# RubensBenevides/Point-Cloud-Registration-with-Global-Refinement

Measured on AMD Instinct MI355X. Metric: point-cloud pairs registered/sec (200k pts, 3 GICP scales), higher is better.
Workload: dtype f32 points+search, f64 normal equations (SURVEY 8a fp column)

## Files before the change

point-cloud-registration-with-global-refinement_amd/csrc/pcr_api.hip:

```cpp
#include <cmath>
#include <cstring>
#include <cstdlib>
#include <cstdio>
#include <atomic>
#include <mutex>
#include <thread>
#include <vector>
#include "pcr_octree.h"

extern "C" int pcr_version(void) { return 220; }

PcrOptions &pcr_options() {
    static PcrOptions o;
    static std::once_flag once;
    std::call_once(once, []() {
        if (const char *e = getenv("PCR_KNN_WAVE")) o.knn_wave = atoi(e);
        if (const char *e = getenv("PCR_KNNW_BUDGET")) o.knnw_budget = atoi(e);
        if (const char *e = getenv("PCR_FENCE_PREP")) o.fence_prep = atoi(e);
        if (getenv("PCR_ICP_VERIFY")) o.icp_verify = 1;
        if (const char *e = getenv("PCR_SPFH_FLOAT64")) o.spfh_float64 = atoi(e);
        if (const char *e = getenv("PCR_RADIUS_LIST_SELECT")) o.radius_list_select = atoi(e);
        if (const char *e = getenv("PCR_FEATNN_MUTUAL")) o.featnn_mutual = atoi(e);
        if (const char *e = getenv("PCR_ICP_SCALES")) o.icp_scales = atoi(e);
        if (const char *e = getenv("PCR_SEARCH_SORT_QUERIES")) o.search_sort_queries = atoi(e);
        if (const char *e = getenv("PCR_FPS_FORM")) o.fps_form = atoi(e);
        if (const char *e = getenv("PCR_FPS_WGS")) o.fps_wgs = atoi(e);
        if (const char *e = getenv("PCR_FPS_TIMEOUT")) o.fps_timeout = atoi(e);
        if (const char *e = getenv("PCR_NFL_FORM")) o.nfl_form = atoi(e);
    });
    return o;
}
PcrCounters &pcr_counters() { static PcrCounters c; return c; }
extern "C" long long pcr_counter(const char *name, int reset) {
    if (!name) return -1;
    PcrCounters &c = pcr_counters();
    std::atomic<long long> *v = !strcmp(name, "fgr_group_barrier_timeouts") ? &c.fgr_group_barrier_timeouts : !strcmp(name, "fgr_group_pool_overflows") ? &c.fgr_group_pool_overflows
                               : !strcmp(name, "fgr_group_pairs_redone_alone") ? &c.fgr_group_pairs_redone_alone : nullptr;
    if (!v) return -1;
    return reset ? v->exchange(0) : v->load();
}
extern "C" int pcr_set_option(const char *name, long long value) {
    if (!name) return PCR_EINVAL;
    PcrOptions &o = pcr_options();
    if (!strcmp(name, "knn_wave")) { o.knn_wave = (int)value; return PCR_OK; }
    if (!strcmp(name, "knnw_budget")) { o.knnw_budget = (int)value; return PCR_OK; }
    if (!strcmp(name, "fence_prep")) { o.fence_prep = (int)value; return PCR_OK; }
    if (!strcmp(name, "icp_verify")) { o.icp_verify = (int)value; return PCR_OK; }
    if (!strcmp(name, "spfh_float64")) { o.spfh_float64 = (int)value; return PCR_OK; }
    if (!strcmp(name, "radius_list_select")) { o.radius_list_select = (int)value; return PCR_OK; }
    if (!strcmp(name, "arena_poison")) { o.arena_poison = (int)value; return PCR_OK; }
    if (!strcmp(name, "featnn_mutual")) { o.featnn_mutual = (int)value; return PCR_OK; }
    if (!strcmp(name, "icp_scales")) { o.icp_scales = (int)value; return PCR_OK; }
    if (!strcmp(name, "search_sort_queries")) { o.search_sort_queries = (int)value; return PCR_OK; }
    if (!strcmp(name, "fps_form")) { o.fps_form = (int)value; return PCR_OK; }
    if (!strcmp(name, "fps_wgs")) { o.fps_wgs = (int)value; return PCR_OK; }
    if (!strcmp(name, "fps_timeout")) { o.fps_timeout = (int)value; return PCR_OK; }
    if (!strcmp(name, "nfl_form")) { o.nfl_form = (int)value; return PCR_OK; }
    return PCR_EINVAL;
}

extern "C" int pcr_create(int device, pcr_context **out) {
    if (!out) return PCR_EINVAL;
    *out = nullptr;
    int count = 0;
    if (hipGetDeviceCount(&count) != hipSuccess || count <= 0) return PCR_EHIP;
    if (device < 0 || device >= count) return PCR_EINVAL;
    if (hipSetDevice(device) != hipSuccess) return PCR_EHIP;
    pcr_context *ctx = new pcr_context();
    ctx->device = device;
    for (int i = 0; i < 2; i++)
        if (hipEventCreateWithFlags(&ctx->side_ev[i], hipEventDisableTiming) != hipSuccess) { delete ctx; return PCR_EHIP; }
    for (int i = 0; i < 8; i++)
        if (hipEventCreateWithFlags(&ctx->lane_ev[i], hipEventDisableTiming) != hipSuccess) { delete ctx; return PCR_EHIP; }
    ctx->pinned_cap = 1 << 16;
    if (hipHostMalloc((void **)&ctx->pinned, ctx->pinned_cap, hipHostMallocDefault) != hipSuccess) { delete ctx; return PCR_EHIP; }
    for (int i = 0; i < 2; i++)
        if (hipEventCreateWithFlags(&ctx->ev[i], hipEventDisableTiming) != hipSuccess) { delete ctx; return PCR_EHIP; }
    for (int i = 0; i < 2; i++)
        if (hipEventCreateWithFlags(&ctx->fence_ev[i], hipEventDisableTiming) != hipSuccess) { delete ctx; return PCR_EHIP; }
    ctx->fence_default = true;
// ... 667 lines not shown
        xyz[2 * g] = p.src_xyz; xyz[2 * g + 1] = p.tgt_xyz; nrm[2 * g] = p.src_normals; nrm[2 * g + 1] = p.tgt_normals;
        n[2 * g] = p.n_src; n[2 * g + 1] = p.n_tgt;
    }
    for (int c = 0; c < C; c++) total += (size_t)n_scales * ((size_t)n[c] + 512) * 1100 + pcr_sort_temp_bytes((size_t)n[c] * n_scales) + (size_t)n[c] * n_scales * 40 + (8u << 20);
    PCR_TRY(pcr_arena_reserve(ctx, total + (16u << 20)));
    std::vector<double> b6((size_t)C * 6);
    PCR_TRY(pcr_dev_bounds_batch(ctx, C, xyz.data(), n.data(), b6.data()));
    std::vector<double> dists((size_t)G * n_scales);
    for (int g = 0; g < G; g++) {
        if (radius_rule == 1) {
            const double *bs = &b6[12 * g], *bt = &b6[12 * g + 6];
            const double r1 = std::pow((bs[3] - bs[0]) * (bs[4] - bs[1]) * (bs[5] - bs[2]), 1.0 / 3.0), r2 = std::pow((bt[3] - bt[0]) * (bt[4] - bt[1]) * (bt[5] - bt[2]), 1.0 / 3.0);
            for (int s = 0; s < n_scales; s++) dists[(size_t)g * n_scales + s] = (r1 + r2) / 2 * std::pow(2.0, -(double)s);
        } else for (int s = 0; s < n_scales; s++) dists[(size_t)g * n_scales + s] = given_dists[s];
        for (int s = 0; s < 8; s++) px[g]->max_distances[s] = s < n_scales ? dists[(size_t)g * n_scales + s] : 0.0;
        for (int s = 0; s < n_scales; s++) if (!(dists[(size_t)g * n_scales + s] > 0.0)) { ctx->err = "max_correspondence_distance <= 0"; return PCR_EINVAL; }
    }
    int *cnt = arena<int>(ctx, (size_t)C * n_scales * 2);
    if (!cnt) return PCR_ENOMEM;
    std::vector<DevCloud> clean;
    bool declined = false;
    PCR_TRY(prep_group_scales(ctx, C, xyz.data(), nrm.data(), n.data(), b6.data(), voxels, n_scales, sor_k, sor_std, normal_k, clean, cnt, &declined));
    if (declined) return 1;
    std::vector<double> T((size_t)G * 16), md((size_t)G);
    std::vector<pcr_result> res((size_t)G);
    std::vector<int32_t *> match((size_t)G);
    for (int g = 0; g < G; g++) {
        memcpy(&T[16 * g], px[g]->base.init_T, 16 * sizeof(double));
        match[g] = arena<int32_t>(ctx, n[2 * g]);
        if (!match[g]) return PCR_ENOMEM;
    }
    int rc_all = 1;
    if (n_scales > 1 && pcr_options().icp_scales.load(std::memory_order_relaxed)) {
        std::vector<const DevCloud *> ss((size_t)G * n_scales), tt((size_t)G * n_scales);
        std::vector<double> mds((size_t)G * n_scales); std::vector<pcr_result> rall((size_t)G * n_scales);
        for (int g = 0; g < G; g++)
            for (int s = 0; s < n_scales; s++) {
                ss[(size_t)g * n_scales + s] = &clean[(size_t)(2 * g) * n_scales + s]; tt[(size_t)g * n_scales + s] = &clean[(size_t)(2 * g + 1) * n_scales + s];
                mds[(size_t)g * n_scales + s] = dists[(size_t)g * n_scales + s];
            }
        rc_all = pcr_dev_gicp_group_scales(ctx, G, n_scales, ss.data(), tt.data(), mds.data(), T.data(), params, rall.data(), match.data());
        if (rc_all != PCR_OK && rc_all != 1) return rc_all;
        if (rc_all == PCR_OK)
            for (int g = 0; g < G; g++) for (int s = 0; s < n_scales; s++) px[g]->base.records[s].icp = rall[(size_t)g * n_scales + s];
    }
    for (int s = 0; s < n_scales && rc_all == 1; s++) {
        std::vector<const DevCloud *> ss((size_t)G), tt((size_t)G);
        for (int g = 0; g < G; g++) { ss[g] = &clean[(size_t)(2 * g) * n_scales + s]; tt[g] = &clean[(size_t)(2 * g + 1) * n_scales + s]; md[g] = dists[(size_t)g * n_scales + s]; }
        PCR_TRY(pcr_dev_gicp_group(ctx, G, ss.data(), tt.data(), md.data(), T.data(), params, res.data(), match.data()));
        for (int g = 0; g < G; g++) { px[g]->base.records[s].icp = res[g]; memcpy(&T[16 * g], res[g].transformation, 16 * sizeof(double)); }
    }
    {
        std::vector<const int32_t *> mm; std::vector<const int *> nn; std::vector<int> cc; std::vector<int32_t *> oo;
        for (int g = 0; g < G; g++)
            if (px[g]->base.correspondences) {
                const DevCloud &last = clean[(size_t)(2 * g) * n_scales + n_scales - 1];
                mm.push_back(match[g]); nn.push_back(last.n); cc.push_back(last.cap); oo.push_back((int32_t *)px[g]->base.correspondences);
            }
        if (!mm.empty()) PCR_TRY(pcr_dev_compact_matches_batch(ctx, (int)mm.size(), mm.data(), nn.data(), cc.data(), oo.data()));
    }
    std::vector<int> h((size_t)C * n_scales * 2);
    PCR_HIP_CHECK(ctx, hipMemcpyAsync(h.data(), cnt, sizeof(int) * h.size(), hipMemcpyDeviceToHost, ctx->stream));
    PCR_HIP_CHECK(ctx, hipStreamSynchronize(ctx->stream));
    for (int g = 0; g < G; g++)
        for (int s = 0; s < n_scales; s++) {
            pcr_scale_record &r = px[g]->base.records[s];
            for (int w = 0; w < 2; w++) { r.n_voxel[w] = h[2 * ((size_t)(2 * g + w) * n_scales + s)]; r.n_clean[w] = h[2 * ((size_t)(2 * g + w) * n_scales + s) + 1]; }
        }
    return PCR_OK;
}

extern "C" int pcr_debug_scale_clouds(pcr_context *ctx, int count, const float *const *xyz, const float *const *normals, const int64_t *n, const double *voxels,
                                      int n_scales, int sor_k, double sor_std, int normal_k, int form, float *const *out_xyz, float *const *out_normals,
                                      int32_t *out_n_voxel, int32_t *out_n_clean) {
    return pcr_api_call(ctx, [&]() -> int {
    if (count < 1 || count > 64 || n_scales < 1 || n_scales > 8 || form < 0 || form > 2 || !xyz || !n || !voxels || !out_xyz || !out_normals || !out_n_voxel || !out_n_clean) return PCR_EINVAL;
    if (sor_k < 1 || !(sor_std > 0.0) || normal_k < 1) { ctx->err = "nb_neighbors < 1, std_ratio <= 0 or knn < 1"; return PCR_EINVAL; }
    for (int s = 0; s < n_scales; s++) if (!(voxels[s] > 0.0)) { ctx->err = "voxel_size <= 0"; return PCR_EINVAL; }
    const size_t K = (size_t)count * n_scales;
    size_t bytes = 16u << 20;
    for (int c = 0; c < count; c++) {
        if (n[c] <= 0 || n[c] > 0x7fffffff / 4 / n_scales || !xyz[c]) return PCR_EINVAL;
        for (int s = 0; s < n_scales; s++) if (!out_xyz[c * n_scales + s] || !out_normals[c * n_scales + s]) return PCR_EINVAL;
        bytes += (size_t)n_scales * ((size_t)n[c] + 512) * 1100 + pcr_sort_temp_bytes((size_t)n[c] * n_scales) + (size_t)n[c] * n_scales * 40 + (8u << 20);
        if (form == 0) bytes += (size_t)n_scales * 2 * pcr_scratch_bytes_for(n[c]);
    }
// ... 498 lines not shown
```

point-cloud-registration-with-global-refinement_amd/csrc/pcr_gicp.hip:

```cpp
#pragma clang fp contract(on)
#include <climits>
#include <cmath>
#include <cstring>
#include <cstdio>
#include <cstdlib>
#include <string>
#include <vector>
#include "pcr_octree.h"
#include "pcr_umeyama.h"
#include "pcr_solve6.h"

#include "pcr_icp_loop.h"
__global__ void k_icp_init(IcpState *st, IcpInit in) { d_icp_init(st, in); }
__global__ void k_icp_init_g(IcpState *st, const IcpInit *in) { d_icp_init(st + blockIdx.x, in[blockIdx.x]); }

template <int OPB>
__device__ static inline int oct_nn_query(const OctView &t, const OctMeta &m, OctStack<OPB> &stk, bool live, float qx, float qy, float qz,
                                          float r2cap, int hint, int ol, int oct, int ob, int *start_pt, float *d1_out, float *d2_out) {
    int best = -1; float bestd = r2cap, secd = r2cap;
    const bool active = live && m.nl >= 1;
    auto visit = [&](int first, int count) {
        int base = first; const int end = first + count;
        float d = 3.4e38f, dd = 3.4e38f; int id = -1;
        while (__ballot(base < end) != 0ull) {
// ... 835 lines not shown
    if (mode == ICP_MODE_P2PL && (p->loss < PCR_LOSS_L2 || p->loss > PCR_LOSS_GM)) { ctx->err = "unknown robust kernel (pcr_loss_kind)"; return PCR_EINVAL; }
    pcr_gicp_params g;
    memset(&g, 0, sizeof g);
    g.loss = mode == ICP_MODE_P2PL ? p->loss : PCR_LOSS_L2; g.loss_k = mode == ICP_MODE_P2PL ? p->loss_k : 1.0; g.epsilon = 1e-3;
    g.relative_fitness = p->relative_fitness; g.relative_rmse = p->relative_rmse; g.max_iteration = p->max_iteration;
    return icp_loop(ctx, src, tgt, max_dist, T0, &g, mode, out, match_dev);
}

int pcr_dev_colored_icp(pcr_context *ctx, const DevCloud *src, const DevCloud *tgt, double max_dist, const double *T0, const pcr_colored_icp_params *p,
                        const double *src_int, const double *tgt_int, const float4 *tgt_grad, pcr_result *out, int32_t *match_dev) {
    if (p->loss < PCR_LOSS_L2 || p->loss > PCR_LOSS_GM) { ctx->err = "unknown robust kernel (pcr_loss_kind)"; return PCR_EINVAL; }
    const double lambda = (p->lambda_geometric >= 0.0 && p->lambda_geometric <= 1.0) ? p->lambda_geometric : 0.968;
    pcr_gicp_params g;
    memset(&g, 0, sizeof g);
    g.loss = p->loss; g.loss_k = p->loss_k; g.epsilon = 1e-3;
    g.relative_fitness = p->relative_fitness; g.relative_rmse = p->relative_rmse; g.max_iteration = p->max_iteration;
    IcpColorArgs c;
    memset(&c, 0, sizeof c);
    c.tgt_grad = tgt_grad; c.tgt_int = tgt_int; c.src_int = src_int; c.sqrt_lg = std::sqrt(lambda); c.sqrt_lp = std::sqrt(1.0 - lambda);
    return icp_loop(ctx, src, tgt, max_dist, T0, &g, ICP_MODE_COLORED, out, match_dev, &c);
}

int pcr_dev_gicp_group(pcr_context *ctx, int G, const DevCloud *const *src, const DevCloud *const *tgt, const double *max_dists, const double *T0,
                       const pcr_gicp_params *p, pcr_result *out, int32_t *const *match_dev) {
    for (int g = 0; g < G; g++) if (!(max_dists[g] > 0.0)) { ctx->err = "max_correspondence_distance <= 0"; return PCR_EINVAL; }
    if (G < 1 || G > ICP_GROUP_MAX) { ctx->err = "GICP group size must be in 1..32"; return PCR_EINVAL; }
    for (int g = 0; g < G; g++) if (!src[g]->nrm || !tgt[g]->nrm) { ctx->err = "GICP needs normals on both clouds"; return PCR_EINVAL; }
    ArenaMark mark(ctx);
    const IcpSwitches &sw = icp_switches();
    int max_cap = 1;
    for (int g = 0; g < G; g++) max_cap = src[g]->cap > max_cap ? src[g]->cap : max_cap;
    const int tile_pts = fused_tile_points(ctx, max_cap, G);
    IcpGroupBuf buf;
    PCR_TRY(icp_group_buf(ctx, &buf));
    IcpArgs *args = buf.args;
    int nblin = 1, nbnn = 1, nbf = 1;
    IcpState *st = arena<IcpState>(ctx, G);
    if (!st) return PCR_ENOMEM;
    for (int g = 0; g < G; g++) {
        const int cap = src[g]->cap > 0 ? src[g]->cap : 1;
        const int tile_g = icp_group_tile(cap, tile_pts) ? icp_group_tile(cap, tile_pts) : tile_pts;
        const IcpGrids n = icp_grids(cap, tile_g);
        nblin = n.nblin > nblin ? n.nblin : nblin; nbnn = n.nbnn > nbnn ? n.nbnn : nbnn; nbf = n.nbf > nbf ? n.nbf : nbf;
        double *partials = arena<double>(ctx, (size_t)(n.nblin > n.nbf ? n.nblin : n.nbf) * NVP);
        int32_t *match = (match_dev && match_dev[g]) ? match_dev[g] : arena<int32_t>(ctx, cap);
        if (!partials || !match) return PCR_ENOMEM;
        IcpArgs &a = args[g]; memset(&a, 0, sizeof a);
        const double max_dist = max_dists[g];
        fill_args(a, src[g], tgt[g], max_dist, p, match, st + g, partials, 0);
        a.tile_rt = icp_group_tile(cap, tile_pts);
        a.ref = arena<float4>(ctx, cap); a.rbest = arena<int32_t>(ctx, cap); a.clist = arena<int4>(ctx, cap);
        if (!a.ref || !a.rbest || !a.clist) return PCR_ENOMEM;
        const double gg = icp_base_gap(max_dist);
        icp_set_search_cap(a, max_dist, gg);
        a.rs_minus_r = (float)gg;
        memcpy(buf.inits[g].T, T0 + 16 * g, sizeof buf.inits[g].T);
    }
    bool grid = false;
    if (sw.grid) {
        std::vector<int> levels((size_t)G); std::vector<GridView> views((size_t)G);
        for (int g = 0; g < G; g++) levels[g] = pcr_grid_level_for(tgt[g], std::sqrt((double)args[g].r2s));
        bool all = true;
        for (int g = 0; g < G; g++) all = all && levels[g] >= 0 && tgt[g]->cap > 0;
        if (all) {
            PCR_TRY(pcr_dev_build_grid_batch(ctx, tgt, levels.data(), G, views.data()));
            grid = true;
            for (int g = 0; g < G; g++) { args[g].grid = views[g]; grid = grid && views[g].tab != nullptr; }
            if (grid)
                for (int g = 0; g < G; g++)
                    icp_set_search_cap(args[g], max_dists[g], icp_gap_for_level(tgt[g], levels[g], max_dists[g], (double)args[g].rs_minus_r));
        }
    }
    if (nbf > 4096) { ctx->err = "GICP group: cloud too large for the fused iteration kernel"; return PCR_EINVAL; }
    PCR_HIP_CHECK(ctx, hipMemcpyAsync(buf.dargs, buf.args, buf.bytes, hipMemcpyHostToDevice, ctx->stream));
    const IcpArgs *dargs = buf.dargs;
    PCR_LAUNCH(ctx, k_icp_init_g, dim3(G), dim3(64), 0, ctx->stream, st, (const IcpInit *)buf.dinits);
    const int max_it = p ? p->max_iteration : 30;
    const bool byval = sw.byval && G <= ICP_BYVAL;
    IcpArgsB hb; memset(&hb, 0, sizeof hb);
    for (int g = 0; g < G && g < ICP_BYVAL; g++) hb.a[g] = args[g];
    auto one_kernel = [&](int launch_index) { return launch_index > 0 && sw.fused; };
    auto enqueue = [&](int launch_index) {
        if (one_kernel(launch_index)) {
            if (byval) PCR_FUSED_LAUNCH(ctx, k_icp_fused_b, grid, tile_pts, dim3(nbf, G), hb);
            else PCR_FUSED_LAUNCH(ctx, k_icp_fused_g, grid, tile_pts, dim3(nbf, G), dargs);
            return;
        }
        if (grid) PCR_LAUNCH(ctx, k_icp_nn_g<true>, dim3(nbnn, G), dim3(ICP_BS), 0, ctx->stream, dargs);
        else PCR_LAUNCH(ctx, k_icp_nn_g<false>, dim3(nbnn, G), dim3(ICP_BS), 0, ctx->stream, dargs);
        PCR_LAUNCH(ctx, k_icp_lin_g, dim3(nblin, G), dim3(LIN_BS), 0, ctx->stream, dargs);
    };
    const void *dargs_v = dargs;
    std::string now;
    { const int w[3] = {nbnn, nblin, nbf}; now.assign((const char *)w, sizeof w); if (byval) now.append((const char *)&hb, sizeof hb); }
    auto graph_for = [&](int which, int len, hipGraphExec_t *exec) -> int {
        const long long kv[6] = {0x47525550ll , G + (grid ? 1000 : 0) + (sw.fused ? 0 : 2000) + (byval ? 4000 : 0), tile_pts, len, which, (long long)(uintptr_t)dargs_v};
        const std::string key((const char *)kv, sizeof kv);
        auto launch_of = [&](int k) { return which == 0 ? k : len + k; };
        IcpGraph *hit = icp_graph_find(ctx, key);
        if (!hit) {
            size_t kernels = 0;
            for (int k = 0; k < len; k++) kernels += one_kernel(launch_of(k)) ? 1 : 2;
            PCR_TRY(icp_graph_capture(ctx, key, len, kernels, [&](int k) { enqueue(launch_of(k)); }, &hit));
            hit->baked = now;
        } else if (hit->baked != now) {
            size_t i = 0;
            for (int k = 0; k < len; k++) {
                const bool one = one_kernel(launch_of(k));
                for (int part = 0; part < (one ? 1 : 2); part++, i++) {
                    if (i >= hit->nodes.size()) { ctx->err = "GICP group: captured chunk shorter than its launch list"; return PCR_EHIP; }
                    hipKernelNodeParams np;
                    PCR_HIP_CHECK(ctx, hipGraphKernelNodeGetParams(hit->nodes[i], &np));
                    void *kp[1];
                    if (one) { np.gridDim = dim3(nbf, G); kp[0] = byval ? (void *)&hb : (void *)&dargs_v; }
                    else { np.gridDim = part == 0 ? dim3(nbnn, G) : dim3(nblin, G); kp[0] = (void *)&dargs_v; }
                    np.kernelParams = kp; np.extra = nullptr;
                    PCR_HIP_CHECK(ctx, hipGraphExecKernelNodeSetParams(hit->exec, hit->nodes[i], &np));
                }
            }
            hit->baked = now;
        }
        *exec = hit->exec;
        return PCR_OK;
    };
    auto issue = [&](int k, int c, bool ragged) -> int {
        hipGraphExec_t ge = nullptr;
        if (sw.graph && !ragged) PCR_TRY(graph_for(k == 0 ? 0 : 1, c, &ge));
        if (ge) PCR_HIP_CHECK(ctx, hipGraphLaunch(ge, ctx->stream));
        else for (int i = 0; i < c; i++) enqueue(k + i);
        return PCR_OK;
    };
    std::vector<IcpState> fin((size_t)G);
    auto judge = [&](const IcpState *s, int, int *next) -> int {
        bool all = true;
        for (int g = 0; g < G; g++) all = all && s[g].done;
        if (all) { fin.assign(s, s + G); *next = 0; return PCR_OK; }
        *next = 1;
        for (int g = 0; g < G; g++)
            if (!s[g].done) { const int l = icp_next_chunk(s[g], args[g].rel_fit, args[g].rel_rmse, sw.chunk, true); *next = l > *next ? l : *next; }
        return PCR_OK;
    };
    IcpPump pump;
    PCR_TRY(pump.init(ctx, st, G));
    PCR_TRY(pump.run(sw.chunk, max_it + 1, issue, judge));
    if (!pump.done) { ctx->err = "GICP group loop ended without a final state"; return PCR_EHIP; }
    PCR_HIP_CHECK(ctx, hipStreamSynchronize(ctx->stream));
    if (ctx->profiling) {
        int longest = 0;
        for (int g = 0; g < G; g++) { icp_prof_add_state(ctx, fin[g]); longest = fin[g].launches > longest ? fin[g].launches : longest; }
        PCR_TRY(pump.add_profile(longest));
    }
    for (int g = 0; g < G; g++) {
        state_to_result(fin[g], &out[g]);
        for (int k = 0; k < 16; k++) if (!std::isfinite(fin[g].T[k])) { ctx->err = "non-finite pose"; return PCR_ENUMERIC; }
    }
    return PCR_OK;
}

int pcr_dev_gicp_group_scales(pcr_context *ctx, int G, int S, const DevCloud *const *src, const DevCloud *const *tgt, const double *max_dists, const double *T0,
                              const pcr_gicp_params *p, pcr_result *out, int32_t *const *match_dev) {
    if (G < 1 || G > ICP_GROUP_MAX || S < 1 || S > 8) return 1;
    const IcpSwitches &sw = icp_switches();
    if (!sw.fused || !sw.grid) return 1;
    if (pcr_options().icp_verify.load(std::memory_order_relaxed)) return 1;
    for (int k = 0; k < G * S; k++) {
        if (!(max_dists[k] > 0.0)) { ctx->err = "max_correspondence_distance <= 0"; return PCR_EINVAL; }
        if (!src[k]->nrm || !tgt[k]->nrm) { ctx->err = "GICP needs normals on both clouds"; return PCR_EINVAL; }
        if (tgt[k]->cap <= 0) return 1;
    }
    int max_cap = 1;
    for (int k = 0; k < G * S; k++) max_cap = src[k]->cap > max_cap ? src[k]->cap : max_cap;
    const int tile_pts = fused_tile_points(ctx, max_cap, G);
    for (int k = 0; k < G * S; k++) {
        const int cap = src[k]->cap > 0 ? src[k]->cap : 1;
        const int tile_k = icp_group_tile(cap, tile_pts) ? icp_group_tile(cap, tile_pts) : tile_pts;
        if (tile_k != LIN_BS) return 1;
    }
    ArenaMark mark(ctx);
    std::vector<int> levels((size_t)G * S); std::vector<GridView> views((size_t)G * S);
    for (int k = 0; k < G * S; k++) {
        IcpArgs base;
        icp_set_search_cap(base, max_dists[k], icp_base_gap(max_dists[k]));
        levels[k] = pcr_grid_level_for(tgt[k], std::sqrt((double)base.r2s));
        if (levels[k] < 0) return 1;
    }
    PCR_TRY(pcr_dev_build_grid_batch(ctx, tgt, levels.data(), G * S, views.data()));
    for (int k = 0; k < G * S; k++) if (!views[k].tab) return 1;
    IcpGroupBuf buf;
    PCR_TRY(icp_group_buf(ctx, &buf));
    IcpArgs *dargs = buf.dargs;
    const void *dargs_v = dargs;
    IcpState *st = arena<IcpState>(ctx, G), *hist = arena<IcpState>(ctx, (size_t)G * S);
    IcpArgs *all_dev = arena<IcpArgs>(ctx, (size_t)G * S);
    if (!st || !hist || !all_dev) return PCR_ENOMEM;
    std::vector<IcpArgs> all((size_t)G * S);
    int nbf = 1;
    for (int g = 0; g < G; g++) {
        int cap_g = 1, rows_g = 1;
        for (int s_ = 0; s_ < S; s_++) {
            const int cap = src[g * S + s_]->cap > 0 ? src[g * S + s_]->cap : 1;
            const int f_ = icp_grids(cap, LIN_BS).nbf;
            nbf = f_ > nbf ? f_ : nbf; cap_g = cap > cap_g ? cap : cap_g; rows_g = f_ > rows_g ? f_ : rows_g;
        }
        double *partials = arena<double>(ctx, (size_t)rows_g * NVP);
        int32_t *match = (match_dev && match_dev[g]) ? match_dev[g] : arena<int32_t>(ctx, cap_g);
        float4 *ref = arena<float4>(ctx, cap_g); int32_t *rbest = arena<int32_t>(ctx, cap_g); int4 *clist = arena<int4>(ctx, cap_g);
        if (!partials || !match || !ref || !rbest || !clist) return PCR_ENOMEM;
        for (int s_ = 0; s_ < S; s_++) {
            const int k = g * S + s_;
            IcpArgs &a = all[k]; memset(&a, 0, sizeof a);
            fill_args(a, src[k], tgt[k], max_dists[k], p, match, st + g, partials, 0);
            a.tile_rt = icp_group_tile(src[k]->cap > 0 ? src[k]->cap : 1, tile_pts);
            a.ref = ref; a.rbest = rbest; a.clist = clist;
            icp_set_search_cap(a, max_dists[k], icp_gap_for_level(tgt[k], levels[k], max_dists[k], icp_base_gap(max_dists[k])));
            a.grid = views[k];
            a.ms_args = all_dev + (size_t)g * S; a.ms_self = dargs + g; a.ms_hist = hist + (size_t)g * S; a.ms_scales = S; a.ms_index = s_;
        }
    }
    if (nbf > 4096) return 1;
    std::vector<IcpArgs> first((size_t)G); std::vector<IcpInit> inits((size_t)G);
    for (int g = 0; g < G; g++) { first[g] = all[(size_t)g * S]; memcpy(inits[g].T, T0 + 16 * g, sizeof inits[g].T); }
    PCR_HIP_CHECK(ctx, hipMemcpyAsync(all_dev, all.data(), sizeof(IcpArgs) * all.size(), hipMemcpyHostToDevice, ctx->stream));
    PCR_HIP_CHECK(ctx, hipMemcpyAsync(dargs, first.data(), sizeof(IcpArgs) * (size_t)G, hipMemcpyHostToDevice, ctx->stream));
    PCR_HIP_CHECK(ctx, hipMemcpyAsync(buf.dinits, inits.data(), sizeof(IcpInit) * (size_t)G, hipMemcpyHostToDevice, ctx->stream));
    PCR_LAUNCH(ctx, k_icp_init_g, dim3(G), dim3(64), 0, ctx->stream, st, (const IcpInit *)buf.dinits);
    auto enqueue_fused = [&](int) { PCR_LAUNCH(ctx, (k_icp_fused_g<LIN_BS, true>), dim3(nbf, G), dim3(FUSED_BS), 0, ctx->stream, (const IcpArgs *)dargs); };
    auto issue = [&](int, int c, bool) -> int {
        IcpGraph *hit = nullptr;
        if (sw.graph) {
            const long long kv[6] = {0x47525053ll , G, LIN_BS, c, nbf, (long long)(uintptr_t)dargs_v};
            const std::string key((const char *)kv, sizeof kv);
            hit = icp_graph_find(ctx, key);
            if (!hit) PCR_TRY(icp_graph_capture(ctx, key, c, 0, enqueue_fused, &hit));
        }
        if (hit) PCR_HIP_CHECK(ctx, hipGraphLaunch(hit->exec, ctx->stream));
        else for (int i = 0; i < c; i++) enqueue_fused(i);
        return PCR_OK;
    };
    const int max_it = p ? p->max_iteration : 30;
    const long long launch_limit = (long long)S * ((long long)max_it + 2) + 4 * sw.chunk + 64;
    IcpPump pump;
    int live_launches = 0;
    auto judge = [&](const IcpState *s, int upto, int *next) -> int {
        bool all_done = true;
        *next = 1;
        for (int g = 0; g < G; g++) {
            if (s[g].done) continue;
            all_done = false;
            const int l = icp_next_chunk(s[g], all[(size_t)g * S].rel_fit, all[(size_t)g * S].rel_rmse, sw.chunk, true);
            *next = l > *next ? l : *next;
        }
        if (all_done) { *next = 0; return PCR_OK; }
        live_launches = upto;
        if (pump.launched > launch_limit) { ctx->err = "GICP group loop (all scales) did not end"; return PCR_EHIP; }
        return PCR_OK;
    };
    PCR_TRY(pump.init(ctx, st, G));
    PCR_TRY(pump.run(sw.chunk, INT_MAX, issue, judge));
    if (!pump.done) { ctx->err = "GICP group loop ended without a final state"; return PCR_EHIP; }
// ... 155 lines not shown
```

point-cloud-registration-with-global-refinement_amd/csrc/pcr_icp_loop.h:

```cpp
#pragma once
#include <cmath>
#include <cstring>
#include <string>
#include <vector>
#include "pcr_octree.h"
#include "pcr_umeyama.h"
#include "pcr_solve6.h"

#define ICP_BS 256
#define NV 30
#define NVP 32
#define LIN_BS 512
#define LIN_MAX_BLOCKS 128

enum { ICP_MODE_GICP = 0, ICP_MODE_EVAL = 1, ICP_MODE_GICP_COV = 2, ICP_MODE_P2PL = 3, ICP_MODE_P2P = 4, ICP_MODE_P2P_SCALED = 5, ICP_MODE_COLORED = 6, ICP_MODE_VGICP = 7,
       ICP_MODE_NDT = 8 };

struct IcpState {
    double T[16];
    double fitness, rmse;
    double sums[NVP];
    long long count;
    int iter;
    int launches;
// ... 255 lines not shown
    if (ctx->icp_graphs.size() >= 48) {
        PCR_HIP_CHECK(ctx, hipStreamSynchronize(ctx->stream));
        (void)hipGraphExecDestroy(ctx->icp_graphs[0].exec);
        if (ctx->icp_graphs[0].graph) (void)hipGraphDestroy(ctx->icp_graphs[0].graph);
        ctx->icp_graphs.erase(ctx->icp_graphs.begin());
    }
    owner.g = nullptr;
    ctx->icp_graphs.push_back(std::move(e));
    *out = &ctx->icp_graphs.back();
    return PCR_OK;
}

struct IcpPump {
    pcr_context *ctx = nullptr;
    const IcpState *st_dev = nullptr; size_t slot_bytes = 0;
    IcpState *slots[2] = {nullptr, nullptr};
    int cur = 0, prev = -1;
    int launched = 0;
    bool done = false;
    std::vector<int> chunk_first, chunk_last;

    int init(pcr_context *c, const IcpState *states_dev, int G) {
        ctx = c; st_dev = states_dev; slot_bytes = sizeof(IcpState) * (size_t)G;
        if (2 * slot_bytes > ctx->pinned_cap) { ctx->err = "ICP loop: pinned window too small"; return PCR_ENOMEM; }
        slots[0] = (IcpState *)ctx->pinned; slots[1] = (IcpState *)(ctx->pinned + slot_bytes);
        return PCR_OK;
    }
    template <class Issue, class Judge>
    int run(int first_len, int total, Issue &&issue, Judge &&judge) {
        int want = first_len;
        for (;;) {
            const int room = total - launched, c = room < want ? (room > 0 ? room : 0) : want;
            if (c > 0) {
                const size_t n = chunk_first.size();
                if (ctx->profiling) {
                    while (ctx->prof_events.size() < 2 * (n + 1)) { hipEvent_t e; PCR_HIP_CHECK(ctx, hipEventCreate(&e)); ctx->prof_events.push_back(e); }
                    PCR_HIP_CHECK(ctx, hipEventRecord(ctx->prof_events[2 * n], ctx->stream));
                }
                PCR_TRY(issue(launched, c, c != want));
                if (ctx->profiling) PCR_HIP_CHECK(ctx, hipEventRecord(ctx->prof_events[2 * n + 1], ctx->stream));
                chunk_first.push_back(launched); chunk_last.push_back(launched + c);
                launched += c;
                PCR_HIP_CHECK(ctx, hipMemcpyAsync(slots[cur], st_dev, slot_bytes, hipMemcpyDeviceToHost, ctx->stream));
                PCR_HIP_CHECK(ctx, hipEventRecord(ctx->ev[cur], ctx->stream));
            }
            if (prev >= 0) {
                PCR_HIP_CHECK(ctx, hipEventSynchronize(ctx->ev[prev]));
// ... 19 lines not shown
```

point-cloud-registration-with-global-refinement_amd/csrc/pcr_internal.h:

```cpp
#pragma once
#include <hip/hip_runtime.h>
#include <stdint.h>
#include <string>
#include <mutex>
#include <cstring>
#include <vector>
#include <atomic>
#include "../../include/pcr_hip.h"

struct PcrOptions { std::atomic<int> knn_wave{-1}, knnw_budget{80}, fence_prep{0}, icp_verify{0}, spfh_float64{0}, radius_list_select{1}, arena_poison{0}, featnn_mutual{1}, icp_scales{1}, search_sort_queries{-1}, fps_form{-1}, fps_wgs{0}, fps_timeout{-1}, nfl_form{1}; };
PcrOptions &pcr_options();
struct PcrCounters { std::atomic<long long> fgr_group_barrier_timeouts{0}, fgr_group_pool_overflows{0}, fgr_group_pairs_redone_alone{0}; };
PcrCounters &pcr_counters();
#define PCR_GROUP_FORMS_MAX_POINTS 400000


struct IcpGraph {
    std::string key;
    hipGraphExec_t exec = nullptr;
    hipGraph_t graph = nullptr;
    std::vector<hipGraphNode_t> nodes;
    std::string baked;
};

struct pcr_context {
    int device = 0;
    hipStream_t stream = nullptr;
    hipStream_t own_stream = nullptr;
    hipStream_t side_stream = nullptr;
    hipStream_t side_stream2 = nullptr;
    hipEvent_t side_ev[2] = {nullptr, nullptr};
    hipEvent_t lane_ev[8] = {};
    char *arena = nullptr;
    size_t arena_cap = 0, arena_off = 0;
    char *aux = nullptr;
// ... 184 lines not shown
                                   double max_dist, const double *T, pcr_result *result, int32_t *correspondences);

size_t pcr_feature_nn_scratch_bytes(int64_t n0, int64_t n1, int prune_mode = -1);
int pcr_feature_nn_mutual(pcr_context *ctx, const float *f0, int n0, const float *f1, int n1, int32_t *out_1to0, int32_t *out_0to1,
                          int prune_mode ,
                          int mutual_only = 0 );

int pcr_feature_nn_mutual_batch(pcr_context *ctx, int G, const float *const *f0, const int *n0, const float *const *f1, const int *n1, int32_t *const *out_1to0,
                                int32_t *const *out_0to1, const int **overflow_dev, int mutual_only = 0);

size_t pcr_feature_corres_scratch_bytes(int64_t ns, int64_t nt);
int pcr_feature_corres(pcr_context *ctx, const float *src_feat, int ns, const float *tgt_feat, int nt, int mutual_filter, int min_rows, int32_t *corres, int64_t *n_out);

int pcr_corres_check(pcr_context *ctx, const int32_t *corres, int64_t n_corres, int64_t n_src, int64_t n_tgt);

struct IcpOutputs { pcr_result res; };
int pcr_dev_gicp(pcr_context *ctx, const DevCloud *src, const DevCloud *tgt, double max_dist, const double *T0,
                 const pcr_gicp_params *p, pcr_result *out, int32_t *match_dev );
int pcr_dev_icp(pcr_context *ctx, const DevCloud *src, const DevCloud *tgt, double max_dist, const double *T0,
                const pcr_icp_params *p, pcr_result *out, int32_t *match_dev );
int pcr_dev_colored_icp(pcr_context *ctx, const DevCloud *src, const DevCloud *tgt, double max_dist, const double *T0, const pcr_colored_icp_params *p,
                        const double *src_int, const double *tgt_int, const float4 *tgt_grad, pcr_result *out, int32_t *match_dev );
void pcr_icp_loop_switches(int *chunk, bool *graph);
int pcr_dev_gicp_group_scales(pcr_context *ctx, int G, int S, const DevCloud *const *src , const DevCloud *const *tgt, const double *max_dists , const double *T0 ,
                              const pcr_gicp_params *p, pcr_result *out , int32_t *const *match_dev );
int pcr_dev_gicp_group(pcr_context *ctx, int G, const DevCloud *const *src, const DevCloud *const *tgt, const double *max_dists , const double *T0 ,
                       const pcr_gicp_params *p, pcr_result *out , int32_t *const *match_dev );
int pcr_dev_linearize_once(pcr_context *ctx, const DevCloud *src, const DevCloud *tgt, double max_dist, const double *T,
                           const pcr_gicp_params *p, double *JTJ36, double *JTr6, double *stats3, int32_t *match_dev);
int pcr_dev_evaluate(pcr_context *ctx, const DevCloud *src, const DevCloud *tgt, double max_dist, const double *T,
                     pcr_result *out, int32_t *match_dev, double *info36 );
int pcr_dev_evaluate_group(pcr_context *ctx, int G, const DevCloud *const *src, const DevCloud *const *tgt, double max_dist, const double *T ,
                           pcr_result *out , int32_t *const *match_dev );
int pcr_dev_compact_matches(pcr_context *ctx, const int32_t *match, const int *n, int cap, const uint32_t *src_perm,
                            const uint32_t *tgt_perm, int32_t *corr_out, int64_t *n_corr);
```

Measured before the change: 725.3.

## Size GICP group grids from live point counts and drop converged pairs

The post-prep point counts are now copied asynchronously into a pinned window right after prep. The GICP group paths poll that window and, once the counts have landed, shrink the fused-kernel grid width from the allocated capacity to the actual point count. In the per-scale path with by-value args, pairs that have converged are also removed from the launch rows. Graph nodes get their grid dimensions updated, alternating between two cached graphs, and new counters track launches, dispatched workgroups and live tiles. The aim is fewer idle workgroups over capacity padding and finished pairs, at the cost of extra graph updates, host polling of volatile memory, and dependence on the pinned-window layout.

```diff
diff --git a/point-cloud-registration-with-global-refinement_amd/csrc/pcr_api.hip b/point-cloud-registration-with-global-refinement_amd/csrc/pcr_api.hip
--- a/point-cloud-registration-with-global-refinement_amd/csrc/pcr_api.hip
+++ b/point-cloud-registration-with-global-refinement_amd/csrc/pcr_api.hip
@@ -27,6 +27,7 @@
         if (const char *e = getenv("PCR_FPS_WGS")) o.fps_wgs = atoi(e);
         if (const char *e = getenv("PCR_FPS_TIMEOUT")) o.fps_timeout = atoi(e);
         if (const char *e = getenv("PCR_NFL_FORM")) o.nfl_form = atoi(e);
+        if (const char *e = getenv("PCR_ICP_LIVE_GRID")) o.icp_live_grid = atoi(e);
     });
     return o;
 }
@@ -35,7 +36,8 @@
     if (!name) return -1;
     PcrCounters &c = pcr_counters();
     std::atomic<long long> *v = !strcmp(name, "fgr_group_barrier_timeouts") ? &c.fgr_group_barrier_timeouts : !strcmp(name, "fgr_group_pool_overflows") ? &c.fgr_group_pool_overflows
-                               : !strcmp(name, "fgr_group_pairs_redone_alone") ? &c.fgr_group_pairs_redone_alone : nullptr;
+                               : !strcmp(name, "fgr_group_pairs_redone_alone") ? &c.fgr_group_pairs_redone_alone : !strcmp(name, "icp_group_launches") ? &c.icp_group_launches
+                               : !strcmp(name, "icp_group_workgroups_dispatched") ? &c.icp_group_workgroups_dispatched : !strcmp(name, "icp_group_tiles_live") ? &c.icp_group_tiles_live : nullptr;
     if (!v) return -1;
     return reset ? v->exchange(0) : v->load();
 }
@@ -56,6 +58,7 @@
     if (!strcmp(name, "fps_wgs")) { o.fps_wgs = (int)value; return PCR_OK; }
     if (!strcmp(name, "fps_timeout")) { o.fps_timeout = (int)value; return PCR_OK; }
     if (!strcmp(name, "nfl_form")) { o.nfl_form = (int)value; return PCR_OK; }
+    if (!strcmp(name, "icp_live_grid")) { o.icp_live_grid = (int)value; return PCR_OK; }
     return PCR_EINVAL;
 }
 
@@ -769,6 +772,11 @@
     bool declined = false;
     PCR_TRY(prep_group_scales(ctx, C, xyz.data(), nrm.data(), n.data(), b6.data(), voxels, n_scales, sor_k, sor_std, normal_k, clean, cnt, &declined));
     if (declined) return 1;
+    const size_t n_cnt = (size_t)C * n_scales * 2;
+    if (n_cnt * sizeof(int) > PCR_PINNED_COUNTS_BYTES || ctx->pinned_cap < 2 * PCR_PINNED_COUNTS_BYTES) { ctx->err = "GICP group: pinned window too small for the counts"; return PCR_ENOMEM; }
+    volatile int *h = (volatile int *)(ctx->pinned + ctx->pinned_cap - PCR_PINNED_COUNTS_BYTES);
+    for (size_t k = 0; k < n_cnt; k++) h[k] = -1;
+    PCR_HIP_CHECK(ctx, hipMemcpyAsync((void *)h, cnt, sizeof(int) * n_cnt, hipMemcpyDeviceToHost, ctx->stream));
     std::vector<double> T((size_t)G * 16), md((size_t)G);
     std::vector<pcr_result> res((size_t)G);
     std::vector<int32_t *> match((size_t)G);
@@ -786,7 +794,8 @@
                 ss[(size_t)g * n_scales + s] = &clean[(size_t)(2 * g) * n_scales + s]; tt[(size_t)g * n_scales + s] = &clean[(size_t)(2 * g + 1) * n_scales + s];
                 mds[(size_t)g * n_scales + s] = dists[(size_t)g * n_scales + s];
             }
-        rc_all = pcr_dev_gicp_group_scales(ctx, G, n_scales, ss.data(), tt.data(), mds.data(), T.data(), params, rall.data(), match.data());
+        const IcpHostCounts hc{h + 1, 4 * n_scales, 2};
+        rc_all = pcr_dev_gicp_group_scales(ctx, G, n_scales, ss.data(), tt.data(), mds.data(), T.data(), params, rall.data(), match.data(), &hc);
         if (rc_all != PCR_OK && rc_all != 1) return rc_all;
         if (rc_all == PCR_OK)
             for (int g = 0; g < G; g++) for (int s = 0; s < n_scales; s++) px[g]->base.records[s].icp = rall[(size_t)g * n_scales + s];
@@ -794,7 +803,8 @@
     for (int s = 0; s < n_scales && rc_all == 1; s++) {
         std::vector<const DevCloud *> ss((size_t)G), tt((size_t)G);
         for (int g = 0; g < G; g++) { ss[g] = &clean[(size_t)(2 * g) * n_scales + s]; tt[g] = &clean[(size_t)(2 * g + 1) * n_scales + s]; md[g] = dists[(size_t)g * n_scales + s]; }
-        PCR_TRY(pcr_dev_gicp_group(ctx, G, ss.data(), tt.data(), md.data(), T.data(), params, res.data(), match.data()));
+        const IcpHostCounts hc{h + 2 * s + 1, 4 * n_scales, 0};
+        PCR_TRY(pcr_dev_gicp_group(ctx, G, ss.data(), tt.data(), md.data(), T.data(), params, res.data(), match.data(), &hc));
         for (int g = 0; g < G; g++) { px[g]->base.records[s].icp = res[g]; memcpy(&T[16 * g], res[g].transformation, 16 * sizeof(double)); }
     }
     {
@@ -804,11 +814,11 @@
                 const DevCloud &last = clean[(size_t)(2 * g) * n_scales + n_scales - 1];
                 mm.push_back(match[g]); nn.push_back(last.n); cc.push_back(last.cap); oo.push_back((int32_t *)px[g]->base.correspondences);
             }
-        if (!mm.empty()) PCR_TRY(pcr_dev_compact_matches_batch(ctx, (int)mm.size(), mm.data(), nn.data(), cc.data(), oo.data()));
-    }
-    std::vector<int> h((size_t)C * n_scales * 2);
-    PCR_HIP_CHECK(ctx, hipMemcpyAsync(h.data(), cnt, sizeof(int) * h.size(), hipMemcpyDeviceToHost, ctx->stream));
-    PCR_HIP_CHECK(ctx, hipStreamSynchronize(ctx->stream));
+        if (!mm.empty()) {
+            PCR_TRY(pcr_dev_compact_matches_batch(ctx, (int)mm.size(), mm.data(), nn.data(), cc.data(), oo.data()));
+            PCR_HIP_CHECK(ctx, hipStreamSynchronize(ctx->stream));
+        }
+    }
     for (int g = 0; g < G; g++)
         for (int s = 0; s < n_scales; s++) {
             pcr_scale_record &r = px[g]->base.records[s];
diff --git a/point-cloud-registration-with-global-refinement_amd/csrc/pcr_gicp.hip b/point-cloud-registration-with-global-refinement_amd/csrc/pcr_gicp.hip
--- a/point-cloud-registration-with-global-refinement_amd/csrc/pcr_gicp.hip
+++ b/point-cloud-registration-with-global-refinement_amd/csrc/pcr_gicp.hip
@@ -881,12 +881,14 @@
 }
 
 int pcr_dev_gicp_group(pcr_context *ctx, int G, const DevCloud *const *src, const DevCloud *const *tgt, const double *max_dists, const double *T0,
-                       const pcr_gicp_params *p, pcr_result *out, int32_t *const *match_dev) {
+                       const pcr_gicp_params *p, pcr_result *out, int32_t *const *match_dev, const IcpHostCounts *counts) {
     for (int g = 0; g < G; g++) if (!(max_dists[g] > 0.0)) { ctx->err = "max_correspondence_distance <= 0"; return PCR_EINVAL; }
     if (G < 1 || G > ICP_GROUP_MAX) { ctx->err = "GICP group size must be in 1..32"; return PCR_EINVAL; }
     for (int g = 0; g < G; g++) if (!src[g]->nrm || !tgt[g]->nrm) { ctx->err = "GICP needs normals on both clouds"; return PCR_EINVAL; }
     ArenaMark mark(ctx);
     const IcpSwitches &sw = icp_switches();
+    const bool live_grid = counts && counts->n && pcr_options().icp_live_grid.load(std::memory_order_relaxed) != 0;
+    std::vector<int> cap_of((size_t)G), tile_of((size_t)G), tiles_of((size_t)G), wide_of((size_t)G);
     int max_cap = 1;
     for (int g = 0; g < G; g++) max_cap = src[g]->cap > max_cap ? src[g]->cap : max_cap;
     const int tile_pts = fused_tile_points(ctx, max_cap, G);
@@ -900,6 +902,7 @@
         const int cap = src[g]->cap > 0 ? src[g]->cap : 1;
         const int tile_g = icp_group_tile(cap, tile_pts) ? icp_group_tile(cap, tile_pts) : tile_pts;
         const IcpGrids n = icp_grids(cap, tile_g);
+        cap_of[g] = cap; tile_of[g] = tile_g; tiles_of[g] = (cap + tile_g - 1) / tile_g; wide_of[g] = n.nbf;
         nblin = n.nblin > nblin ? n.nblin : nblin; nbnn = n.nbnn > nbnn ? n.nbnn : nbnn; nbf = n.nbf > nbf ? n.nbf : nbf;
         double *partials = arena<double>(ctx, (size_t)(n.nblin > n.nbf ? n.nblin : n.nbf) * NVP);
         int32_t *match = (match_dev && match_dev[g]) ? match_dev[g] : arena<int32_t>(ctx, cap);
@@ -936,12 +939,44 @@
     PCR_LAUNCH(ctx, k_icp_init_g, dim3(G), dim3(64), 0, ctx->stream, st, (const IcpInit *)buf.dinits);
     const int max_it = p ? p->max_iteration : 30;
     const bool byval = sw.byval && G <= ICP_BYVAL;
-    IcpArgsB hb; memset(&hb, 0, sizeof hb);
-    for (int g = 0; g < G && g < ICP_BYVAL; g++) hb.a[g] = args[g];
+    const bool live_rows = live_grid && byval;
+    std::vector<int> rows((size_t)G);
+    for (int g = 0; g < G; g++) rows[g] = g;
+    IcpArgsB hb;
+    int ny = G;
+    long long tiles_rows = 0;
+    auto set_rows = [&]() {
+        memset(&hb, 0, sizeof hb);
+        ny = (int)rows.size(); tiles_rows = 0; nbf = 8;
+        for (int j = 0; j < ny; j++) {
+            if (byval) hb.a[j] = args[rows[j]];
+            nbf = wide_of[rows[j]] > nbf ? wide_of[rows[j]] : nbf;
+            tiles_rows += tiles_of[rows[j]];
+        }
+    };
+    bool sized = false;
+    auto size_by_counts = [&]() {
+        if (!counts || !counts->n || sized) return;
+        for (int g = 0; g < G; g++) if (counts->n[(size_t)g * counts->pair_stride] < 0) return;
+        if (live_grid) { nblin = 1; nbnn = 1; }
+        for (int g = 0; g < G; g++) {
+            const int c = counts->n[(size_t)g * counts->pair_stride];
+            const int ns_g = c < 1 ? 1 : (c > cap_of[g] ? cap_of[g] : c);
+            const IcpGrids w = icp_grids(ns_g, tile_of[g]);
+            tiles_of[g] = (ns_g + tile_of[g] - 1) / tile_of[g];
+            if (!live_grid) continue;
+            wide_of[g] = w.nbf;
+            nblin = w.nblin > nblin ? w.nblin : nblin; nbnn = w.nbnn > nbnn ? w.nbnn : nbnn;
+        }
+        sized = true;
+        set_rows();
+    };
+    set_rows();
+    size_by_counts();
     auto one_kernel = [&](int launch_index) { return launch_index > 0 && sw.fused; };
     auto enqueue = [&](int launch_index) {
         if (one_kernel(launch_index)) {
-            if (byval) PCR_FUSED_LAUNCH(ctx, k_icp_fused_b, grid, tile_pts, dim3(nbf, G), hb);
+            if (byval) PCR_FUSED_LAUNCH(ctx, k_icp_fused_b, grid, tile_pts, dim3(nbf, ny), hb);
             else PCR_FUSED_LAUNCH(ctx, k_icp_fused_g, grid, tile_pts, dim3(nbf, G), dargs);
             return;
         }
@@ -950,10 +985,11 @@
         PCR_LAUNCH(ctx, k_icp_lin_g, dim3(nblin, G), dim3(LIN_BS), 0, ctx->stream, dargs);
     };
     const void *dargs_v = dargs;
-    std::string now;
-    { const int w[3] = {nbnn, nblin, nbf}; now.assign((const char *)w, sizeof w); if (byval) now.append((const char *)&hb, sizeof hb); }
+    int side = 0;
     auto graph_for = [&](int which, int len, hipGraphExec_t *exec) -> int {
-        const long long kv[6] = {0x47525550ll , G + (grid ? 1000 : 0) + (sw.fused ? 0 : 2000) + (byval ? 4000 : 0), tile_pts, len, which, (long long)(uintptr_t)dargs_v};
+        std::string now;
+        { const int w[4] = {nbnn, nblin, nbf, ny}; now.assign((const char *)w, sizeof w); if (byval) now.append((const char *)&hb, sizeof hb); }
+        const long long kv[6] = {0x47525550ll , G + (grid ? 1000 : 0) + (sw.fused ? 0 : 2000) + (byval ? 4000 : 0) + (live_grid ? 8000 + 8000 * side : 0), tile_pts, len, which, (long long)(uintptr_t)dargs_v};
         const std::string key((const char *)kv, sizeof kv);
         auto launch_of = [&](int k) { return which == 0 ? k : len + k; };
         IcpGraph *hit = icp_graph_find(ctx, key);
@@ -971,7 +1007,7 @@
                     hipKernelNodeParams np;
                     PCR_HIP_CHECK(ctx, hipGraphKernelNodeGetParams(hit->nodes[i], &np));
                     void *kp[1];
-                    if (one) { np.gridDim = dim3(nbf, G); kp[0] = byval ? (void *)&hb : (void *)&dargs_v; }
+                    if (one) { np.gridDim = byval ? dim3(nbf, ny) : dim3(nbf, G); kp[0] = byval ? (void *)&hb : (void *)&dargs_v; }
                     else { np.gridDim = part == 0 ? dim3(nbnn, G) : dim3(nblin, G); kp[0] = (void *)&dargs_v; }
                     np.kernelParams = kp; np.extra = nullptr;
                     PCR_HIP_CHECK(ctx, hipGraphExecKernelNodeSetParams(hit->exec, hit->nodes[i], &np));
@@ -983,10 +1019,18 @@
         return PCR_OK;
     };
     auto issue = [&](int k, int c, bool ragged) -> int {
+        size_by_counts();
         hipGraphExec_t ge = nullptr;
         if (sw.graph && !ragged) PCR_TRY(graph_for(k == 0 ? 0 : 1, c, &ge));
         if (ge) PCR_HIP_CHECK(ctx, hipGraphLaunch(ge, ctx->stream));
         else for (int i = 0; i < c; i++) enqueue(k + i);
+        side ^= 1;
+        long long fused_launches = 0;
+        for (int i = 0; i < c; i++) fused_launches += one_kernel(k + i) ? 1 : 0;
+        PcrCounters &tally = pcr_counters();
+        tally.icp_group_launches += fused_launches;
+        tally.icp_group_workgroups_dispatched += fused_launches * (long long)nbf * (byval ? ny : G);
+        tally.icp_group_tiles_live += fused_launches * tiles_rows;
         return PCR_OK;
     };
     std::vector<IcpState> fin((size_t)G);
@@ -994,6 +1038,12 @@
         bool all = true;
         for (int g = 0; g < G; g++) all = all && s[g].done;
         if (all) { fin.assign(s, s + G); *next = 0; return PCR_OK; }
+        size_by_counts();
+        if (live_rows) {
+            size_t keep = 0;
+            for (size_t j = 0; j < rows.size(); j++) if (!s[rows[j]].done) rows[keep++] = rows[j];
+            if (keep != rows.size()) { rows.resize(keep); set_rows(); }
+        }
         *next = 1;
         for (int g = 0; g < G; g++)
             if (!s[g].done) { const int l = icp_next_chunk(s[g], args[g].rel_fit, args[g].rel_rmse, sw.chunk, true); *next = l > *next ? l : *next; }
@@ -1017,8 +1067,9 @@
 }
 
 int pcr_dev_gicp_group_scales(pcr_context *ctx, int G, int S, const DevCloud *const *src, const DevCloud *const *tgt, const double *max_dists, const double *T0,
-                              const pcr_gicp_params *p, pcr_result *out, int32_t *const *match_dev) {
+                              const pcr_gicp_params *p, pcr_result *out, int32_t *const *match_dev, const IcpHostCounts *counts) {
     if (G < 1 || G > ICP_GROUP_MAX || S < 1 || S > 8) return 1;
+    const bool live_grid = counts && counts->n && pcr_options().icp_live_grid.load(std::memory_order_relaxed) != 0;
     const IcpSwitches &sw = icp_switches();
     if (!sw.fused || !sw.grid) return 1;
     if (pcr_options().icp_verify.load(std::memory_order_relaxed)) return 1;
@@ -1054,6 +1105,7 @@
     if (!st || !hist || !all_dev) return PCR_ENOMEM;
     std::vector<IcpArgs> all((size_t)G * S);
     int nbf = 1;
+    long long tiles_group = 0;
     for (int g = 0; g < G; g++) {
         int cap_g = 1, rows_g = 1;
         for (int s_ = 0; s_ < S; s_++) {
@@ -1061,6 +1113,7 @@
             const int f_ = icp_grids(cap, LIN_BS).nbf;
             nbf = f_ > nbf ? f_ : nbf; cap_g = cap > cap_g ? cap : cap_g; rows_g = f_ > rows_g ? f_ : rows_g;
         }
+        tiles_group += (cap_g + LIN_BS - 1) / LIN_BS;
         double *partials = arena<double>(ctx, (size_t)rows_g * NVP);
         int32_t *match = (match_dev && match_dev[g]) ? match_dev[g] : arena<int32_t>(ctx, cap_g);
         float4 *ref = arena<float4>(ctx, cap_g); int32_t *rbest = arena<int32_t>(ctx, cap_g); int4 *clist = arena<int4>(ctx, cap_g);
@@ -1084,16 +1137,56 @@
     PCR_HIP_CHECK(ctx, hipMemcpyAsync(buf.dinits, inits.data(), sizeof(IcpInit) * (size_t)G, hipMemcpyHostToDevice, ctx->stream));
     PCR_LAUNCH(ctx, k_icp_init_g, dim3(G), dim3(64), 0, ctx->stream, st, (const IcpInit *)buf.dinits);
     auto enqueue_fused = [&](int) { PCR_LAUNCH(ctx, (k_icp_fused_g<LIN_BS, true>), dim3(nbf, G), dim3(FUSED_BS), 0, ctx->stream, (const IcpArgs *)dargs); };
+    bool sized = false;
+    auto size_by_counts = [&]() {
+        if (!counts || !counts->n || sized) return;
+        for (int k = 0; k < G * S; k++) if (counts->n[(size_t)(k / S) * counts->pair_stride + (size_t)(k % S) * counts->scale_stride] < 0) return;
+        if (live_grid) nbf = 8;
+        tiles_group = 0;
+        for (int g = 0; g < G; g++) {
+            int tiles_g = 1;
+            for (int s_ = 0; s_ < S; s_++) {
+                const int cap = src[g * S + s_]->cap > 0 ? src[g * S + s_]->cap : 1, c = counts->n[(size_t)g * counts->pair_stride + (size_t)s_ * counts->scale_stride];
+                const int ns_k = c < 1 ? 1 : (c > cap ? cap : c);
+                const int w_ = icp_grids(ns_k, LIN_BS).nbf, t_ = (ns_k + LIN_BS - 1) / LIN_BS;
+                if (live_grid) nbf = w_ > nbf ? w_ : nbf;
+                tiles_g = t_ > tiles_g ? t_ : tiles_g;
+            }
+            tiles_group += tiles_g;
+        }
+        sized = true;
+    };
+    size_by_counts();
+    int side = 0;
     auto issue = [&](int, int c, bool) -> int {
+        size_by_counts();
+        const std::string now((const char *)&nbf, sizeof nbf);
         IcpGraph *hit = nullptr;
         if (sw.graph) {
-            const long long kv[6] = {0x47525053ll , G, LIN_BS, c, nbf, (long long)(uintptr_t)dargs_v};
+            const long long kv[6] = {0x47525053ll , G, LIN_BS, c, side, (long long)(uintptr_t)dargs_v};
             const std::string key((const char *)kv, sizeof kv);
             hit = icp_graph_find(ctx, key);
-            if (!hit) PCR_TRY(icp_graph_capture(ctx, key, c, 0, enqueue_fused, &hit));
+            if (!hit) {
+                PCR_TRY(icp_graph_capture(ctx, key, c, (size_t)c, enqueue_fused, &hit));
+                hit->baked = now;
+            } else if (hit->baked != now) {
+                for (size_t i = 0; i < hit->nodes.size(); i++) {
+                    hipKernelNodeParams np;
+                    PCR_HIP_CHECK(ctx, hipGraphKernelNodeGetParams(hit->nodes[i], &np));
+                    void *kp[1] = {(void *)&dargs_v};
+                    np.gridDim = dim3(nbf, G); np.kernelParams = kp; np.extra = nullptr;
+                    PCR_HIP_CHECK(ctx, hipGraphExecKernelNodeSetParams(hit->exec, hit->nodes[i], &np));
+                }
+                hit->baked = now;
+            }
         }
         if (hit) PCR_HIP_CHECK(ctx, hipGraphLaunch(hit->exec, ctx->stream));
         else for (int i = 0; i < c; i++) enqueue_fused(i);
+        side ^= 1;
+        PcrCounters &tally = pcr_counters();
+        tally.icp_group_launches += c;
+        tally.icp_group_workgroups_dispatched += (long long)c * nbf * G;
+        tally.icp_group_tiles_live += (long long)c * tiles_group;
         return PCR_OK;
     };
     const int max_it = p ? p->max_iteration : 30;
diff --git a/point-cloud-registration-with-global-refinement_amd/csrc/pcr_icp_loop.h b/point-cloud-registration-with-global-refinement_amd/csrc/pcr_icp_loop.h
--- a/point-cloud-registration-with-global-refinement_amd/csrc/pcr_icp_loop.h
+++ b/point-cloud-registration-with-global-refinement_amd/csrc/pcr_icp_loop.h
@@ -301,7 +301,7 @@
 
     int init(pcr_context *c, const IcpState *states_dev, int G) {
         ctx = c; st_dev = states_dev; slot_bytes = sizeof(IcpState) * (size_t)G;
-        if (2 * slot_bytes > ctx->pinned_cap) { ctx->err = "ICP loop: pinned window too small"; return PCR_ENOMEM; }
+        if (2 * slot_bytes + PCR_PINNED_COUNTS_BYTES > ctx->pinned_cap) { ctx->err = "ICP loop: pinned window too small"; return PCR_ENOMEM; }
         slots[0] = (IcpState *)ctx->pinned; slots[1] = (IcpState *)(ctx->pinned + slot_bytes);
         return PCR_OK;
     }
diff --git a/point-cloud-registration-with-global-refinement_amd/csrc/pcr_internal.h b/point-cloud-registration-with-global-refinement_amd/csrc/pcr_internal.h
--- a/point-cloud-registration-with-global-refinement_amd/csrc/pcr_internal.h
+++ b/point-cloud-registration-with-global-refinement_amd/csrc/pcr_internal.h
@@ -8,9 +8,9 @@
 #include <atomic>
 #include "../../include/pcr_hip.h"
 
-struct PcrOptions { std::atomic<int> knn_wave{-1}, knnw_budget{80}, fence_prep{0}, icp_verify{0}, spfh_float64{0}, radius_list_select{1}, arena_poison{0}, featnn_mutual{1}, icp_scales{1}, search_sort_queries{-1}, fps_form{-1}, fps_wgs{0}, fps_timeout{-1}, nfl_form{1}; };
+struct PcrOptions { std::atomic<int> knn_wave{-1}, knnw_budget{80}, fence_prep{0}, icp_verify{0}, spfh_float64{0}, radius_list_select{1}, arena_poison{0}, featnn_mutual{1}, icp_scales{1}, search_sort_queries{-1}, fps_form{-1}, fps_wgs{0}, fps_timeout{-1}, nfl_form{1}, icp_live_grid{1}; };
 PcrOptions &pcr_options();
-struct PcrCounters { std::atomic<long long> fgr_group_barrier_timeouts{0}, fgr_group_pool_overflows{0}, fgr_group_pairs_redone_alone{0}; };
+struct PcrCounters { std::atomic<long long> fgr_group_barrier_timeouts{0}, fgr_group_pool_overflows{0}, fgr_group_pairs_redone_alone{0}, icp_group_launches{0}, icp_group_workgroups_dispatched{0}, icp_group_tiles_live{0}; };
 PcrCounters &pcr_counters();
 #define PCR_GROUP_FORMS_MAX_POINTS 400000
 
@@ -241,10 +241,14 @@
 int pcr_dev_colored_icp(pcr_context *ctx, const DevCloud *src, const DevCloud *tgt, double max_dist, const double *T0, const pcr_colored_icp_params *p,
                         const double *src_int, const double *tgt_int, const float4 *tgt_grad, pcr_result *out, int32_t *match_dev );
 void pcr_icp_loop_switches(int *chunk, bool *graph);
+struct IcpHostCounts { const volatile int *n; int pair_stride, scale_stride; };
+#define PCR_PINNED_COUNTS_BYTES 4096
 int pcr_dev_gicp_group_scales(pcr_context *ctx, int G, int S, const DevCloud *const *src , const DevCloud *const *tgt, const double *max_dists , const double *T0 ,
-                              const pcr_gicp_params *p, pcr_result *out , int32_t *const *match_dev );
+                              const pcr_gicp_params *p, pcr_result *out , int32_t *const *match_dev ,
+                              const IcpHostCounts *counts = nullptr );
 int pcr_dev_gicp_group(pcr_context *ctx, int G, const DevCloud *const *src, const DevCloud *const *tgt, const double *max_dists , const double *T0 ,
-                       const pcr_gicp_params *p, pcr_result *out , int32_t *const *match_dev );
+                       const pcr_gicp_params *p, pcr_result *out , int32_t *const *match_dev ,
+                       const IcpHostCounts *counts = nullptr );
 int pcr_dev_linearize_once(pcr_context *ctx, const DevCloud *src, const DevCloud *tgt, double max_dist, const double *T,
                            const pcr_gicp_params *p, double *JTJ36, double *JTr6, double *stats3, int32_t *match_dev);
 int pcr_dev_evaluate(pcr_context *ctx, const DevCloud *src, const DevCloud *tgt, double max_dist, const double *T,
```

Result: no change. 723.8 (-0.2%).
